# grantjr1842/delayed-streams-modeling

Measured on AMD Instinct MI355X. Metric: real-time stream throughput, stt-1b-en_fr @ bs=64 per GPU (Mimi encode + LM decode per 80 ms frame), higher is better.
Workload: dtype bf16 weights + bf16 KV, f32 activations as three exact bf16 pieces, f32 accumulate (v_mfma_f32_16x16x32_bf16); 1 GPU; stt-1b-en_fr batch=64 streaming, ring KV cache full (750 frames), Mimi encode + LM decode HIP path; streams_per_gpu=64, parallelism=replicas x1 (independent stream batches, no per-step collective), streams=encoder stream || 2 LM group stream(s)

## Files before the change

### delayed-streams-modeling_amd/csrc/dsm_engine.hip

```cpp
#include <hip/hip_runtime.h>

#include <cmath>
#include <cstdarg>
#include <cstdio>
#include <cstdlib>
#include <cstring>
#include <atomic>
#include <mutex>
#include <shared_mutex>
#include <string>
#include <set>
#include <vector>

#include "../../include/dsm.h"
#include "dsm_config_presets.h"
#include "dsm_kernels.h"
#include "dsm_numerics.h"
#include "dsm_safetensors.h"

static thread_local std::string g_create_error;

#define HIPCHK_E(eng, expr)                                                                         \
  do {                                                                                              \
    hipError_t _e = (expr);                                                                         \
// ... 181 lines not shown
  int attn_nt = 1;
  bool fuse_front = false;
  int smallk_loop = 1;
  int smallk_min_tiles = 1024;
  int smallk_mt = 4;
  int chunk_loop_min_tiles = 384;
  bool bx3u = true;
  bool wk_norm = false;
  int wk_gate_max_chunks = 4;
  bool bx3u_m64 = true;
  bool bx3u_late = true;
  int attn_unr = 0;
  bool attn_small = true;
  int prio_hi = 0;
  bool serialize_groups = false;
  hipEvent_t ev_codes_consumed = nullptr;
  bool codes_consumed_valid = false;
  hipEvent_t ev_join = nullptr, ev_a = nullptr, ev_b = nullptr, ev_c = nullptr, ev_d = nullptr;
  MimiW mimi_w;
  MimiState mimi[2];
  std::atomic<bool> mimi1_ready{false};
  std::mutex mimi1_mu;
  MimiDecState dec;
  float* h_pcm_out = nullptr;
  LmW lm_w;
  LmState lm;
  std::vector<void*> allocs;
  std::string err;
  float* h_pcm = nullptr;
  float* h_pcm1 = nullptr;
  uint8_t* h_mask = nullptr;
  uint32_t *h_codes = nullptr, *h_text = nullptr;
// ... 666 lines not shown
  }
  int MT = a.M > 32 ? 4 : (a.M > 16 ? 2 : 1);
  while (MT > 1 && (long)gx * chunks * ((a.M + 16 * MT - 1) / (16 * MT)) < 256) MT /= 2;
  if (MT == 4 && e->bx3u && e->bx3u_m64 && e->dot_mode == 1 && sizeof(WT) == 2 && chunks > 1 && a.chunk_loop == 0 && a.M <= 64 &&
      (long)gx * chunks <= 256 && EPI == EPI_STORE)
    MT = 2;
  const bool smallk = e->smallk_loop && chunks == 1 && a.chunk_loop == 0 && (long)gx * ((a.M + 63) / 64) >= e->smallk_min_tiles &&
                      !(e->dot_mode == 1 && sizeof(WT) == 2);
  if (smallk && e->smallk_mt < MT) MT = e->smallk_mt;
  auto ok4 = [](const RowMap& m) { return m.ld % 4 == 0 && m.bstride % 4 == 0; };
  a.vec = (a.N % 4 == 0) && (!a.Y || ok4(a.ymap)) && (!a.Y2 || ok4(a.y2map)) && (!a.res || ok4(a.rmap));
  a.ws_ntiles = (((NT - 1) * a.nt_stride) >> 4) + gx * 4;
  const int mtiles = (a.M + 15) / 16;
  if (chunks > 1) {
    const int wsid = e->sid(st);
    size_t need = (size_t)chunks * mtiles * a.ws_ntiles * 256 * sizeof(float);
    if (need > e->gemm_ws_cap[wsid]) {
      if (e->capturing) {
        e->capture_failed = true;
        e->set_error("split-K workspace grew during a graph capture");
        return DSM_ERR_STATE;
      }
      e->ws_gen += 1;
      HIPCHK(hipStreamSynchronize(st));
      if (e->gemm_ws[wsid]) HIPCHK(hipFree(e->gemm_ws[wsid]));
      e->gemm_ws[wsid] = nullptr;
      e->gemm_ws_cap[wsid] = 0;
      void* p = nullptr;
      HIPCHK(hipMalloc(&p, need));
      e->gemm_ws[wsid] = reinterpret_cast<float*>(p);
      e->gemm_ws_cap[wsid] = need;
    }
    a.ws = e->gemm_ws[wsid];
  }
  dim3 grid(gx, chunks, (a.M + 16 * MT - 1) / (16 * MT));
  const bool nt2 = NT == 1 && e->dot_mode == 1 && sizeof(WT) == 2 && e->bx3_nt2 && a.chunk_loop > 1 && MT == 4 &&
                   (EPI == EPI_STORE || EPI == EPI_QKV) && a.N % 128 == 0 && (long)(a.N / 128) * grid.z >= e->bx3_nt2_min;
  if (nt2) {
    grid.x = a.N / 128;
    a.wg_cols = 128;
    a.nt_stride = 64;
  }
  a.ts = e->timeline ? e->dev_ts_slot(e->tag_gemm[e->sid(st)], e->sid(st), 1, 2) : nullptr;
  const int ph = e->prof_begin(e->tag_gemm[e->sid(st)], st);
  const bool bx3 = e->dot_mode == 1 && sizeof(WT) == 2;
  const bool roll = (a.chunk_loop > 1 && e->roll_prefetch) || smallk;
  constexpr int DMAX = LoopDepth<WT, NT>::MAX;
  const bool deep = DMAX == 4 && e->loop_depth == 4 && !smallk;
// ... 202 lines not shown
```

### delayed-streams-modeling_amd/csrc/dsm_engine_api.inc

```

namespace {

template <typename KVT, int HD, int T>
int launch_attn_t(dsm_engine* e, hipStream_t st, float* out, const float* q, const void* k, const void* v,
                  const uint32_t* start_pos, const uint8_t* active, int B, int H, int ctx, int d, const AttnFused& fq) {
  size_t lds = sizeof(float) * ((size_t)T * ctx + 4 * T * HD + 16);
  if ((long)B * H >= 2048 && (size_t)2 * ctx * HD * sizeof(KVT) >= (size_t)256 * 1024) lds += e->attn_lds_pad;
  if (lds > 64 * 1024) {
    static size_t allowed = 0;
    if (lds > allowed) {
      HIPCHK(hipFuncSetAttribute(reinterpret_cast<const void*>(&attn_kernel<KVT, HD, T, 8>), hipFuncAttributeMaxDynamicSharedMemorySize, (int)lds));
      HIPCHK(hipFuncSetAttribute(reinterpret_cast<const void*>(&attn_kernel<KVT, HD, T, 4>), hipFuncAttributeMaxDynamicSharedMemorySize, (int)lds));
      allowed = lds;
    }
  }
  const int tag = e->tag_attn[e->sid(st)];
  if (T == 1 && HD == 64 && ctx <= 32 && e->attn_small) {
    const int ph = e->prof_begin(tag, st);
    hipLaunchKernelGGL((attn_small_kernel<KVT, 64>), dim3((B * H + 3) / 4), dim3(256), 0, st, out, q, reinterpret_cast<const KVT*>(k),
                       reinterpret_cast<const KVT*>(v), start_pos, active, B * H, H, ctx, d, fq);
    e->prof_end(ph, st);
    HIPCHK(hipGetLastError());
    return 0;
  }
// ... 402 lines not shown
  const dsm_asr_config& c = e->cfg;
  LmState& s = e->lm;
  const LmW& w = e->lm_w;
  LmState::Group& grp = s.groups[g];
  const int B = e->B, d = c.lm.d_model, b0 = grp.b0, nb = grp.nb;
  e->tag_gemm[e->sid(st)] = DSM_PROF_GEMM_LM;
  e->tag_attn[e->sid(st)] = DSM_PROF_ATTN_LM;
  uint8_t* gmask = s.gmask + b0;
  float* x = s.x + (size_t)b0 * d;
  const int hid = w.tr.hidden;
  float *xn = s.xn + (size_t)b0 * d, *q = s.q + (size_t)b0 * d, *att = s.att + (size_t)b0 * d, *gg = s.g + (size_t)b0 * hid;
  float* hidden = s.hidden + (size_t)b0 * d;
  int rc;
  if (c.kv_bf16)
    rc = transformer_forward<uint16_t, uint16_t>(e, st, w.tr, grp.view, x, xn, q, att, gg, nb, 1, gmask, nullptr,
                                                 plain_map(1, 1), w.out_norm, hidden, phase);
  else
    rc = transformer_forward<uint16_t, float>(e, st, w.tr, grp.view, x, xn, q, att, gg, nb, 1, gmask, nullptr,
                                              plain_map(1, 1), w.out_norm, hidden, phase);
  if (rc || phase == 1) return rc;
  float* logits = s.logits + (size_t)b0 * c.text_out_vocab_size;
  {
    GemmArgs a = base_args(w.text_linear, hidden, plain_map(nb, d), nb);
    a.Y = logits; a.ymap = plain_map(nb, c.text_out_vocab_size);
    if ((rc = gemm_store<uint16_t>(e, st, a))) return rc;
  }
  if (c.temperature > 0.0f)
    hipLaunchKernelGGL(lm_gumbel_kernel, dim3(nb), dim3(256), 0, st, logits, c.text_out_vocab_size, c.temperature,
                       s.rng_key + (size_t)b0 * 8, s.rng_pos + b0, d_text_out + b0, s.text_token + b0, s.first_step + b0, gmask);
  else
    hipLaunchKernelGGL(lm_argmax_kernel, dim3(nb), dim3(256), 0, st, logits, c.text_out_vocab_size, d_text_out + b0,
                       s.text_token + b0, s.first_step + b0, gmask);
  HIPCHK(hipGetLastError());
  if (c.extra_heads_num > 0 && d_prs_out) {
    const int ehw = c.extra_heads_num * c.extra_heads_dim;
    float* eh = s.eh + (size_t)b0 * ehw;
    GemmArgs a = base_args(w.extra_heads, hidden, plain_map(nb, d), nb);
    a.Y = eh; a.ymap = plain_map(nb, ehw);
    if ((rc = gemm_store<uint16_t>(e, st, a))) return rc;
    int n = nb * c.extra_heads_num;
    hipLaunchKernelGGL(extra_heads_kernel, dim3((n + 255) / 256), dim3(256), 0, st, eh, d_prs_out + b0, nb,
                       c.extra_heads_num, c.extra_heads_dim, B);
    HIPCHK(hipGetLastError());
  }
  return 0;
}

int lm_group_head(dsm_engine* e, hipStream_t st, int g, const uint32_t* d_codes, const uint8_t* d_mask, bool with_prefix) {
  const dsm_asr_config& c = e->cfg;
  LmState& s = e->lm;
  const LmW& w = e->lm_w;
  LmState::Group& grp = s.groups[g];
  const int d = c.lm.d_model, b0 = grp.b0, nb = grp.nb, nc = c.audio_codebooks;
  uint8_t* gmask = s.gmask + b0;
  HIPCHK(hipMemcpyAsync(gmask, d_mask + b0, (size_t)nb, hipMemcpyDeviceToDevice, st));
  float* x = s.x + (size_t)b0 * d;
  hipLaunchKernelGGL(lm_input_kernel, dim3(nb, (d + 511) / 512), dim3(256), 0, st, x, w.text_emb, w.audio_emb,
                     d_codes + (size_t)b0 * nc, s.next_cb + (size_t)b0 * nc, s.text_token + b0, s.first_step + b0, gmask, nc, d,
                     c.audio_vocab_size, (uint32_t)c.audio_vocab_size - 1, (uint32_t)c.text_in_vocab_size - 1);
  hipLaunchKernelGGL(lm_next_codebooks_kernel, dim3((nb * nc + 255) / 256), dim3(256), 0, st, d_codes + (size_t)b0 * nc,
                     s.next_cb + (size_t)b0 * nc, gmask, nb, nc);
  HIPCHK(hipGetLastError());
  if (g > 0) HIPCHK(hipEventRecord(e->ev_grp_in[g], st));
  if (with_prefix)
    if (int rc = lm_group_body(e, st, g, nullptr, nullptr, 1)) return rc;
  return 0;
}

int lm_group_rest(dsm_engine* e, hipStream_t st, int g, uint32_t* d_text_out, float* d_prs_out, bool after_prefix) {
  const uint64_t key = (uint64_t)e->sid(st) ^ ((uint64_t)(uintptr_t)d_text_out << 3) ^ ((uint64_t)(uintptr_t)d_prs_out * 0x9E3779B97F4A7C15ull) ^
                       (after_prefix ? 0x8000000000000000ull : 0ull);
  return run_captured(e, e->g_grp[g], st, key, [&] { return lm_group_body(e, st, g, d_text_out, d_prs_out, after_prefix ? 2 : 0); });
}

int wait_group_inputs(dsm_engine* e) {
  if (!e->grp_busy) return 0;
  for (size_t g = 1; g < e->lm.groups.size(); ++g) HIPCHK(hipStreamWaitEvent(e->s_model, e->ev_grp_in[g], 0));
  return 0;
// ... 186 lines not shown
  for (auto& ps : e->pipe) {
    if (ps.h_pcm) (void)hipHostFree(ps.h_pcm);
    if (ps.h_mask) (void)hipHostFree(ps.h_mask);
    if (ps.ev_done) (void)hipEventDestroy(ps.ev_done);
    if (ps.ev_consumed) (void)hipEventDestroy(ps.ev_consumed);
  }
  for (float* p : e->gemm_ws)
    if (p) (void)hipFree(p);
  if (e->h_pcm) (void)hipHostFree(e->h_pcm);
  if (e->h_pcm1) (void)hipHostFree(e->h_pcm1);
  if (e->h_mask) (void)hipHostFree(e->h_mask);
  if (e->h_codes) (void)hipHostFree(e->h_codes);
  if (e->h_text) (void)hipHostFree(e->h_text);
  if (e->h_prs) (void)hipHostFree(e->h_prs);
  if (e->h_pcm_out) (void)hipHostFree(e->h_pcm_out);
  for (hipEvent_t ev : {e->ev_join, e->ev_codes_consumed, e->ev_a, e->ev_b, e->ev_c, e->ev_d})
    if (ev) (void)hipEventDestroy(ev);
  for (auto& r : e->prof_recs) { (void)hipEventDestroy(r.a); (void)hipEventDestroy(r.b); }
  for (hipEvent_t ev : e->prof_pool) (void)hipEventDestroy(ev);
  for (int g = 0; g < dsm_engine::kMaxGroups; ++g) {
    if (e->ev_grp_in[g]) (void)hipEventDestroy(e->ev_grp_in[g]);
    if (e->ev_grp_done[g]) (void)hipEventDestroy(e->ev_grp_done[g]);
    if (e->ev_stagger[g]) (void)hipEventDestroy(e->ev_stagger[g]);
    if (e->s_grp[g]) (void)hipStreamDestroy(e->s_grp[g]);
  }
  if (e->ev_fork) (void)hipEventDestroy(e->ev_fork);
  if (e->s_enc) (void)hipStreamDestroy(e->s_enc);
  if (e->s_model) (void)hipStreamDestroy(e->s_model);
  delete e;
}

// ... 95 lines not shown
  if (const char* env = getenv("DSM_WK_GATE_CHUNKS")) e->wk_gate_max_chunks = atoi(env);
  if (const char* env = getenv("DSM_FUSE_FRONT")) e->fuse_front = atoi(env) != 0;
  if (const char* env = getenv("DSM_ATTN_NT")) e->attn_nt = atoi(env);
  if (const char* env = getenv("DSM_SMALLK_LOOP")) e->smallk_loop = atoi(env);
  if (const char* env = getenv("DSM_SMALLK_MIN")) e->smallk_min_tiles = atoi(env);
  if (const char* env = getenv("DSM_SMALLK_MT")) { const int v = atoi(env); if (v == 1 || v == 2 || v == 4) e->smallk_mt = v; }
  if (c.dot_mode == 1) e->attn_lds_pad = 40000;
  if (const char* env = getenv("DSM_ATTN_LDS_PAD")) e->attn_lds_pad = (size_t)atol(env);
  if (const char* env = getenv("DSM_ENC_CUS")) e->enc_cus = atoi(env);
  if (const char* env = getenv("DSM_BX3_NT2")) e->bx3_nt2 = atoi(env) != 0;
  if (const char* env = getenv("DSM_BX3_NT2_MIN")) e->bx3_nt2_min = atoi(env);
  if (const char* env = getenv("DSM_LM_CUS_EXCL")) e->lm_cus_excl = atoi(env) != 0;
  if (int rc = make_stream(e, &e->s_enc, prio_lo, 1)) return rc;
  if (int rc = make_stream(e, &e->s_model, prio_hi, 2)) return rc;
  HIPCHK(hipEventCreateWithFlags(&e->ev_join, hipEventDisableTiming));
  HIPCHK(hipEventCreateWithFlags(&e->ev_codes_consumed, hipEventDisableTiming));
  HIPCHK(hipEventCreate(&e->ev_a));
  HIPCHK(hipEventCreate(&e->ev_b));
  HIPCHK(hipEventCreate(&e->ev_c));
  HIPCHK(hipEventCreate(&e->ev_d));
  const int B = batch_size, d = c.lm.d_model;
  if (attach_arena) {
    e->arena = const_cast<char*>(reinterpret_cast<const char*>(attach_arena));
    e->arena_size = attach_bytes;
    e->arena_owned = false;
    e->manifest.assign(attach_manifest, attach_manifest + attach_manifest_bytes);
    e->manifest_pos = 0;
    e->arena_off = 0;
    e->wmode = dsm_engine::W_ATTACH;
    if (int rc = load_all_weights(e, nullptr, nullptr)) return rc;
    if (e->arena_off != e->arena_size || e->manifest_pos != e->manifest.size()) {
// ... 79 lines not shown
      int nb = std::min(blocks * 16, B - b0);
      LmState::Group& grp = s.groups[g];
      grp.b0 = b0;
      grp.nb = nb;
      grp.view = s.tr;
      for (int l = 0; l < c.lm.num_layers; ++l) {
        grp.view.k[l] = (char*)s.tr.k[l] + (size_t)b0 * H * c.lm.context * hd * kv_elem;
        grp.view.v[l] = (char*)s.tr.v[l] + (size_t)b0 * H * c.lm.context * hd * kv_elem;
      }
      grp.view.pos = s.tr.pos + b0;
      grp.view.idx = s.tr.idx + b0;
      grp.view.start_pos = s.tr.start_pos + b0;
      grp.view.widx = s.tr.widx + b0;
      grp.view.rope_cs = s.tr.rope_cs + (size_t)b0 * hd;
      b0 += nb;
      if (g > 0) {
        if (int rc = make_stream(e, &e->s_grp[g], e->prio_hi, 2)) return rc;
        HIPCHK(hipEventCreateWithFlags(&e->ev_grp_in[g], hipEventDisableTiming));
        HIPCHK(hipEventCreateWithFlags(&e->ev_grp_done[g], hipEventDisableTiming));
      }
    }
    HIPCHK(hipEventCreateWithFlags(&e->ev_fork, hipEventDisableTiming));
    for (int g = 0; g + 1 < G; ++g) HIPCHK(hipEventCreateWithFlags(&e->ev_stagger[g], hipEventDisableTiming));
  }
  {
    long n = (long)B * c.audio_codebooks;
    hipLaunchKernelGGL(fill_u32_kernel, dim3((unsigned)((n + 255) / 256)), dim3(256), 0, e->s_model, s.next_cb,
                       (uint32_t)c.audio_vocab_size - 1, n);
    hipLaunchKernelGGL(fill_u32_kernel, dim3((unsigned)((B + 255) / 256)), dim3(256), 0, e->s_model, s.text_token,
                       (uint32_t)c.text_in_vocab_size - 1, (long)B);
    HIPCHK(hipGetLastError());
    HIPCHK(hipMemsetAsync(s.first_step, 1, B, e->s_model));
  }
// ... 404 lines not shown
  std::lock_guard<std::mutex> lk(e->err_mu);
  snprintf(out->capture_error, sizeof out->capture_error, "%s", e->capture_error.c_str());
}

int dsm_get_metrics(dsm_engine* e, dsm_metrics* out) {
  if (!e || !out) return DSM_ERR_INVALID;
  *out = e->metrics;
  fill_graph_metrics(e, out);
  return 0;
}

int dsm_mimi_encode_step_dev(dsm_engine* e, const float* d_pcm, const uint8_t* d_mask, uint32_t* d_codes_out) {
  if (!e || !d_pcm || !d_mask) return DSM_ERR_INVALID;
  HIPCHK(hipSetDevice(e->device));
  ApiShared api(e);
  if (e->codes_consumed_valid) HIPCHK(hipStreamWaitEvent(e->s_enc, e->ev_codes_consumed, 0));
  if (int rc = upload_pcm(e, 0, e->s_enc, d_pcm, hipMemcpyDeviceToDevice)) return rc;
  HIPCHK(hipMemcpyAsync(e->mimi[0].mask, d_mask, (size_t)e->B, hipMemcpyDeviceToDevice, e->s_enc));
  if (int rc = mimi_encode(e, 0, e->s_enc)) return rc;
  if (d_codes_out)
    HIPCHK(hipMemcpyAsync(d_codes_out, e->mimi[0].codes, sizeof(uint32_t) * (size_t)e->B * e->cfg.mimi.quantizer_n_q,
                          hipMemcpyDeviceToDevice, e->s_enc));
  HIPCHK(hipEventRecord(e->ev_join, e->s_enc));
  e->metrics.steps_encode += 1;
  return 0;
}

int dsm_asr_step_tokens_dev(dsm_engine* e, const uint32_t* d_codes, const uint8_t* d_mask, uint32_t* d_text_tokens_out,
                            float* d_vad_prs_out) {
  if (!e || !d_mask) return DSM_ERR_INVALID;
  HIPCHK(hipSetDevice(e->device));
  ApiShared api(e);
  if (int rc = wait_group_inputs(e)) return rc;
  HIPCHK(hipMemcpyAsync(e->lm.mask, d_mask, (size_t)e->B, hipMemcpyDeviceToDevice, e->s_model));
  const uint32_t* codes = d_codes;
  if (!codes) {
    HIPCHK(hipStreamWaitEvent(e->s_model, e->ev_join, 0));
    HIPCHK(hipMemcpyAsync(e->lm.codes_in, e->mimi[0].codes, sizeof(uint32_t) * (size_t)e->B * e->cfg.audio_codebooks,
                          hipMemcpyDeviceToDevice, e->s_model));
    HIPCHK(hipEventRecord(e->ev_codes_consumed, e->s_model));
    e->codes_consumed_valid = true;
    codes = e->lm.codes_in;
  }
  if (int rc = lm_step(e, e->s_model, codes, e->lm.mask, d_text_tokens_out ? d_text_tokens_out : e->lm.text_out,
                       e->cfg.extra_heads_num > 0 ? (d_vad_prs_out ? d_vad_prs_out : e->lm.prs) : nullptr))
    return rc;
  e->metrics.steps_lm += 1;
  e->model_step_idx += 1;
  return 0;
}

int dsm_asr_step_pcm_dev(dsm_engine* e, const float* d_pcm, const uint8_t* d_mask, uint32_t* d_codes_out,
                         uint32_t* d_text_tokens_out, float* d_vad_prs_out) {
  if (!e || !d_pcm || !d_mask) return DSM_ERR_INVALID;
  HIPCHK(hipSetDevice(e->device));
  if (int rc = ensure_model_side_mimi(e)) return rc;
  ApiShared api(e);
  hipStream_t st = e->s_model;
  if (int rc = wait_group_inputs(e)) return rc;
// ... 192 lines not shown
```

### delayed-streams-modeling_amd/csrc/dsm_kernels.h

```cpp
#pragma once
#include <hip/hip_runtime.h>
#include <stdint.h>
#include "dsm_numerics.h"
#include "dsm_sampling.h"

typedef float f32x4 __attribute__((ext_vector_type(4)));
typedef short dsm_bf16x8 __attribute__((ext_vector_type(8)));

__device__ __forceinline__ float wave_sum64(float v) {
#pragma unroll
  for (int off = 32; off >= 1; off >>= 1) v = v + __shfl_xor(v, off, 64);
  return v;
}

enum { EPI_STORE = 0, EPI_QKV = 1, EPI_GATE = 2, EPI_RVQ = 3 };

struct RowMap {
  long bstride;
  int rpb;
  int ld;
  int toff;
  __host__ __device__ long off(int m) const { return (long)(m / rpb) * bstride + (long)((m % rpb) + toff) * ld; }
};

// ... 27 lines not shown
  float* ws;
  int ws_ntiles;
  int defer_reduce;
  int chunk_loop;
  const float* norm_w;
  const float* norm_b;
  float* norm_out;
  float norm_eps;
  int norm_rms;
  int wk_hint;
  const float* pre_norm_w;
  const float* pre_norm_b;
  float pre_norm_eps;
  int pre_norm_rms;
  unsigned long long* ts;
};

template <typename WT>
__device__ __forceinline__ const WT* dsm_wbase(const GemmArgs& a, const WT* W, int n0, int r, int q) {
  if (sizeof(WT) == 2 && a.wpacked) return W + ((long)(n0 >> 4) * (a.Kpad >> 5)) * 512 + (q * 16 + r) * 8;
  return W + (long)(n0 + r) * a.Kpad + 8 * q;
}
template <typename WT>
__device__ __forceinline__ int dsm_wstep(const GemmArgs& a) { return (sizeof(WT) == 2 && a.wpacked) ? 16 : 1; }

__device__ __forceinline__ void launch_stamp_begin(unsigned long long* ts) {
  if (!ts || threadIdx.x != 0) return;
  const unsigned lin = blockIdx.x + gridDim.x * (blockIdx.y + gridDim.y * blockIdx.z);
  if (lin < 128) atomicMin(&ts[0], wall_clock64());
}
// ... 1243 lines not shown
  }
  __syncthreads();
  if (rope_cs) {
    const int half = hd / 2;
    for (int e = threadIdx.x; e < T * half; e += blockDim.x) {
      int t = e / half, i = e % half;
      float ang = (float)(s_pos_after + (uint32_t)t) * inv_freq[i];
      float s, c;
      dsm_sincosf(ang, &s, &c);
      rope_cs[((long)(b * T + t) * half + i) * 2] = c;
      rope_cs[((long)(b * T + t) * half + i) * 2 + 1] = s;
    }
  }
}

__global__ void lm_input_kernel(float* __restrict__ x, const uint16_t* __restrict__ text_emb,
                                const uint16_t* __restrict__ audio_emb ,
                                const uint32_t* __restrict__ codes , uint32_t* __restrict__ next_cb,
                                const uint32_t* __restrict__ text_token, const uint8_t* __restrict__ first_step,
                                const uint8_t* __restrict__ active, int nc, int d, int audio_vocab,
                                uint32_t pad_tok, uint32_t start_tok) {
  const int b = blockIdx.x;
  __shared__ uint32_t toks[64];
  const bool first = first_step[b] != 0;
  if (threadIdx.x < nc) toks[threadIdx.x] = first ? pad_tok : next_cb[b * nc + threadIdx.x];
  __syncthreads();
  const uint32_t tt = first ? start_tok : text_token[b];
  const int j = (blockIdx.y * blockDim.x + threadIdx.x) * 2;
  if (j < d) {
    uint32_t t2 = *reinterpret_cast<const uint32_t*>(text_emb + (long)tt * d + j);
    float e0 = __uint_as_float(t2 << 16), e1 = __uint_as_float(t2 & 0xFFFF0000u);
    for (int i = 0; i < nc; ++i) {
      uint32_t a2 = *reinterpret_cast<const uint32_t*>(audio_emb + ((long)i * audio_vocab + toks[i]) * d + j);
      e0 = e0 + __uint_as_float(a2 << 16);
      e1 = e1 + __uint_as_float(a2 & 0xFFFF0000u);
    }
    *reinterpret_cast<float2*>(x + (long)b * d + j) = make_float2(e0, e1);
  }
}

__global__ void lm_next_codebooks_kernel(const uint32_t* __restrict__ codes, uint32_t* __restrict__ next_cb,
                                         const uint8_t* __restrict__ active, int B, int nc) {
  const int i = blockIdx.x * blockDim.x + threadIdx.x;
  if (i < B * nc && active[i / nc]) next_cb[i] = codes[i];
}

__device__ inline int block_argmax_first(const float* __restrict__ lg, int V) {
  float bv = -DSM_INF_F;
  int bi = 0x7FFFFFFF;
  for (int j = threadIdx.x; j < V; j += blockDim.x) {
    float v = lg[j];
    if (v > bv || (v == bv && j < bi)) { bv = v; bi = j; }
  }
  __shared__ float sv[256];
  __shared__ int si[256];
  sv[threadIdx.x] = bv;
  si[threadIdx.x] = bi;
  __syncthreads();
  for (int off = blockDim.x / 2; off >= 1; off >>= 1) {
    if ((int)threadIdx.x < off) {
      float ov = sv[threadIdx.x + off];
      int oi = si[threadIdx.x + off];
      if (ov > sv[threadIdx.x] || (ov == sv[threadIdx.x] && oi < si[threadIdx.x])) {
        sv[threadIdx.x] = ov;
        si[threadIdx.x] = oi;
      }
    }
    __syncthreads();
  }
  const int r = si[0] == 0x7FFFFFFF ? 0 : si[0];
  __syncthreads();
  return r;
}

__global__ void lm_argmax_kernel(const float* __restrict__ logits, int V, uint32_t* __restrict__ text_out,
                                 uint32_t* __restrict__ text_token, uint8_t* __restrict__ first_step,
                                 const uint8_t* __restrict__ active) {
  const int b = blockIdx.x;
  const uint32_t tok = (uint32_t)block_argmax_first(logits + (long)b * V, V);
  if (threadIdx.x == 0) {
    text_out[b] = tok;
    if (active[b]) {
      text_token[b] = tok;
      first_step[b] = 0;
    }
  }
}

__global__ void lm_gumbel_kernel(const float* __restrict__ logits, int V, float temperature, const uint32_t* __restrict__ rng_key,
                                 unsigned long long* __restrict__ rng_pos, uint32_t* __restrict__ text_out,
                                 uint32_t* __restrict__ text_token, uint8_t* __restrict__ first_step,
                                 const uint8_t* __restrict__ active) {
  const int b = blockIdx.x;
  const float* lg = logits + (long)b * V;
  uint32_t key[8];
#pragma unroll
  for (int i = 0; i < 8; ++i) key[i] = rng_key[b * 8 + i];
  const unsigned long long pos = rng_pos[b];
  float bv = -DSM_INF_F;
  int bi = 0x7FFFFFFF;
  const int nblk = (V + 15) >> 4;
  for (int blk = threadIdx.x; blk < nblk; blk += blockDim.x) {
    uint32_t w[16];
    dsm_chacha_block(key, (pos >> 4) + (unsigned long long)blk, 12, w);
#pragma unroll
    for (int i = 0; i < 16; ++i) {
      const int j = 16 * blk + i;
      if (j < V) {
        const float v = dsm_gumbel_value(lg[j], w[i], temperature);
        if (v > bv || (v == bv && j < bi)) { bv = v; bi = j; }
      }
    }
  }
  __shared__ float sv[256];
  __shared__ int si[256];
  sv[threadIdx.x] = bv;
  si[threadIdx.x] = bi;
  __syncthreads();
  for (int off = blockDim.x / 2; off >= 1; off >>= 1) {
    if ((int)threadIdx.x < off) {
      const float ov = sv[threadIdx.x + off];
      const int oi = si[threadIdx.x + off];
      if (ov > sv[threadIdx.x] || (ov == sv[threadIdx.x] && oi < si[threadIdx.x])) { sv[threadIdx.x] = ov; si[threadIdx.x] = oi; }
    }
    __syncthreads();
  }
  if (threadIdx.x == 0) {
    const uint32_t tok = si[0] == 0x7FFFFFFF ? 0u : (uint32_t)si[0];
    text_out[b] = tok;
    if (active[b]) {
      text_token[b] = tok;
      first_step[b] = 0;
      rng_pos[b] = pos + 16ull * (unsigned long long)nblk;
    }
  }
}

__global__ void tts_input_kernel(float* __restrict__ x, const uint16_t* __restrict__ text_emb,
                                 const uint16_t* __restrict__ audio_emb ,
                                 const int32_t* __restrict__ tokens, int nc, int d, int audio_vocab) {
  const int b = blockIdx.x;
  __shared__ int32_t toks[72];
  if ((int)threadIdx.x < 1 + nc) toks[threadIdx.x] = tokens[b * (1 + nc) + threadIdx.x];
  __syncthreads();
  const int j = (blockIdx.y * blockDim.x + threadIdx.x) * 2;
  if (j < d) {
    uint32_t t2 = *reinterpret_cast<const uint32_t*>(text_emb + (long)toks[0] * d + j);
    float e0 = __uint_as_float(t2 << 16), e1 = __uint_as_float(t2 & 0xFFFF0000u);
    for (int i = 0; i < nc; ++i) {
      const int32_t t = toks[1 + i];
// ... 247 lines not shown
    lat[(long)b * S + k] = tok;
    const uint32_t nt = (forced[b] && k > 0) ? pad : tok;
    last_tok[b] = nt;
    s_next = nt;
  }
  if (!next.x) return;
  }
  __syncthreads();
  const uint32_t t = s_next;
  for (int j = 0; j < next.rps; ++j) {
    if (j > 0) __syncthreads();
    dep_head_row(next, b * next.rps + j, t, hred);
  }
}

__global__ void extra_heads_kernel(const float* __restrict__ eh , float* __restrict__ prs, int B,
                                   int nh, int dim, int prs_stride ) {
  int i = blockIdx.x * blockDim.x + threadIdx.x;
  if (i >= B * nh) return;
  int b = i / nh, h = i % nh;
  const float* lg = eh + ((long)b * nh + h) * dim;
  float m = lg[0];
  for (int k = 1; k < dim; ++k) m = lg[k] > m ? lg[k] : m;
  float sum = 0.0f, e0 = 0.0f;
  for (int k = 0; k < dim; ++k) {
    float e = dsm_expf(lg[k] - m);
    if (k == 0) e0 = e;
    sum = sum + e;
  }
  prs[(long)h * prs_stride + b] = e0 / sum;
}

struct SeanetFrontArgs {
  const float* cat_init;
  const float *w0, *b0;
  const float *w1, *b1;
  const float *w2, *b2;
  float* cat_ra;
  float* cat_down;
  int ld0, ld1, ld2;
  int T, S0, Sd;
};

template <int TM>
constexpr size_t seanet_front_lds() { return sizeof(float) * ((TM + 2) * 64 + TM * 64 + TM * 32 + (TM + 2 + 7 - 1)); }
// ... 270 lines not shown
```

Measured before the change: 1817 x realtime (stream-seconds of audio per wall second).

## Fuse LM head input, KV bookkeeping, first norm; defer split-K reduce into sampling

Combines the LM input embedding, next-codebook copy, mask copy, position/ring-index update, rope sin/cos and the first layer's pre-norm into one per-row lm_head_kernel. The text and extra-heads GEMMs skip their split-K reduction; the argmax/Gumbel and softmax kernels sum the partial chunks themselves from a shared workspace at offsets set by ws_base. The encoder's code-copy handoff is also dropped: the LM reads Mimi codes directly, and the encoder waits on per-group input events instead. The aim is fewer kernel launches and device copies per step, at the cost of more complex workspace management and heavier sampling kernels.

After: 1813 x realtime (stream-seconds of audio per wall second), median of 2. Within noise of the previous version (-0.2%).

```diff
diff --git a/delayed-streams-modeling_amd/csrc/dsm_engine.hip b/delayed-streams-modeling_amd/csrc/dsm_engine.hip
--- a/delayed-streams-modeling_amd/csrc/dsm_engine.hip
+++ b/delayed-streams-modeling_amd/csrc/dsm_engine.hip
@@ -219,8 +219,7 @@
   bool attn_small = true;
   int prio_hi = 0;
   bool serialize_groups = false;
-  hipEvent_t ev_codes_consumed = nullptr;
-  bool codes_consumed_valid = false;
+  std::atomic<bool> enc_codes_read{false};
   hipEvent_t ev_join = nullptr, ev_a = nullptr, ev_b = nullptr, ev_c = nullptr, ev_d = nullptr;
   MimiW mimi_w;
   MimiState mimi[2];
@@ -917,7 +916,7 @@
   const int mtiles = (a.M + 15) / 16;
   if (chunks > 1) {
     const int wsid = e->sid(st);
-    size_t need = (size_t)chunks * mtiles * a.ws_ntiles * 256 * sizeof(float);
+    size_t need = ((size_t)a.ws_base + (size_t)chunks * mtiles * a.ws_ntiles * 256) * sizeof(float);
     if (need > e->gemm_ws_cap[wsid]) {
       if (e->capturing) {
         e->capture_failed = true;
@@ -926,15 +925,20 @@
       }
       e->ws_gen += 1;
       HIPCHK(hipStreamSynchronize(st));
+      void* p = nullptr;
+      HIPCHK(hipMalloc(&p, need));
+      if (a.ws_base > 0 && e->gemm_ws[wsid])
+      {
+        HIPCHK(hipMemcpyAsync(p, e->gemm_ws[wsid], std::min((size_t)a.ws_base * sizeof(float), e->gemm_ws_cap[wsid]), hipMemcpyDeviceToDevice, st));
+        HIPCHK(hipStreamSynchronize(st));
+      }
       if (e->gemm_ws[wsid]) HIPCHK(hipFree(e->gemm_ws[wsid]));
       e->gemm_ws[wsid] = nullptr;
       e->gemm_ws_cap[wsid] = 0;
-      void* p = nullptr;
-      HIPCHK(hipMalloc(&p, need));
       e->gemm_ws[wsid] = reinterpret_cast<float*>(p);
       e->gemm_ws_cap[wsid] = need;
     }
-    a.ws = e->gemm_ws[wsid];
+    a.ws = e->gemm_ws[wsid] + a.ws_base;
   }
   dim3 grid(gx, chunks, (a.M + 16 * MT - 1) / (16 * MT));
   const bool nt2 = NT == 1 && e->dot_mode == 1 && sizeof(WT) == 2 && e->bx3_nt2 && a.chunk_loop > 1 && MT == 4 &&
diff --git a/delayed-streams-modeling_amd/csrc/dsm_engine_api.inc b/delayed-streams-modeling_amd/csrc/dsm_engine_api.inc
--- a/delayed-streams-modeling_amd/csrc/dsm_engine_api.inc
+++ b/delayed-streams-modeling_amd/csrc/dsm_engine_api.inc
@@ -440,33 +440,72 @@
   int rc;
   if (c.kv_bf16)
     rc = transformer_forward<uint16_t, uint16_t>(e, st, w.tr, grp.view, x, xn, q, att, gg, nb, 1, gmask, nullptr,
-                                                 plain_map(1, 1), w.out_norm, hidden, phase);
+                                                 plain_map(1, 1), w.out_norm, hidden, phase, nullptr, true);
   else
     rc = transformer_forward<uint16_t, float>(e, st, w.tr, grp.view, x, xn, q, att, gg, nb, 1, gmask, nullptr,
-                                              plain_map(1, 1), w.out_norm, hidden, phase);
+                                              plain_map(1, 1), w.out_norm, hidden, phase, nullptr, true);
   if (rc || phase == 1) return rc;
-  float* logits = s.logits + (size_t)b0 * c.text_out_vocab_size;
+  const int V = c.text_out_vocab_size, mt16 = (nb + 15) / 16;
+  float* logits = s.logits + (size_t)b0 * V;
+  LogitSrc tsrc{}, hsrc{};
+  tsrc.rps = hsrc.rps = 1;
+  long ws_used = 0;
+  bool tdefer = false;
   {
     GemmArgs a = base_args(w.text_linear, hidden, plain_map(nb, d), nb);
-    a.Y = logits; a.ymap = plain_map(nb, c.text_out_vocab_size);
+    a.Y = logits; a.ymap = plain_map(nb, V);
+    a.defer_reduce = (a.Kpad > DSM_KC && a.K % 32 == 0 && !a.bias && V % 4 == 0) ? 1 : 0;
     if ((rc = gemm_store<uint16_t>(e, st, a))) return rc;
-  }
-  if (c.temperature > 0.0f)
-    hipLaunchKernelGGL(lm_gumbel_kernel, dim3(nb), dim3(256), 0, st, logits, c.text_out_vocab_size, c.temperature,
-                       s.rng_key + (size_t)b0 * 8, s.rng_pos + b0, d_text_out + b0, s.text_token + b0, s.first_step + b0, gmask);
-  else
-    hipLaunchKernelGGL(lm_argmax_kernel, dim3(nb), dim3(256), 0, st, logits, c.text_out_vocab_size, d_text_out + b0,
-                       s.text_token + b0, s.first_step + b0, gmask);
-  HIPCHK(hipGetLastError());
-  if (c.extra_heads_num > 0 && d_prs_out) {
+    if (a.defer_reduce) {
+      tdefer = true;
+      tsrc.ld = (long)a.ws_ntiles * 16;
+      tsrc.cstride = (long)mt16 * 16 * tsrc.ld;
+      tsrc.chunks = (a.Kpad + DSM_KC - 1) / DSM_KC;
+      tsrc.store = logits;
+      ws_used = tsrc.chunks * tsrc.cstride;
+    } else {
+      tsrc.rows = logits;
+    }
+  }
+  const bool heads = c.extra_heads_num > 0 && d_prs_out;
+  if (heads) {
     const int ehw = c.extra_heads_num * c.extra_heads_dim;
     float* eh = s.eh + (size_t)b0 * ehw;
     GemmArgs a = base_args(w.extra_heads, hidden, plain_map(nb, d), nb);
     a.Y = eh; a.ymap = plain_map(nb, ehw);
+    a.defer_reduce = (a.Kpad > DSM_KC && a.K % 32 == 0 && !a.bias) ? 1 : 0;
+    a.ws_base = ws_used;
     if ((rc = gemm_store<uint16_t>(e, st, a))) return rc;
-    int n = nb * c.extra_heads_num;
-    hipLaunchKernelGGL(extra_heads_kernel, dim3((n + 255) / 256), dim3(256), 0, st, eh, d_prs_out + b0, nb,
-                       c.extra_heads_num, c.extra_heads_dim, B);
+    if (a.defer_reduce) {
+      hsrc.ws = a.ws;
+      hsrc.ld = (long)a.ws_ntiles * 16;
+      hsrc.cstride = (long)mt16 * 16 * hsrc.ld;
+      hsrc.chunks = (a.Kpad + DSM_KC - 1) / DSM_KC;
+      hsrc.store = eh;
+    } else {
+      hsrc.rows = eh;
+    }
+  }
+  if (tdefer) tsrc.ws = e->gemm_ws[e->sid(st)];
+  const size_t lds = sizeof(float) * (size_t)((V + 3) & ~3);
+  if (lds > 160 * 1024) {
+    e->set_error("text_out_vocab_size=%d: a logits row does not fit in LDS", V);
+    return DSM_ERR_INVALID;
+  }
+  if (lds > 64 * 1024) {
+    static size_t allowed = 0;
+    if (lds > allowed) {
+      HIPCHK(hipFuncSetAttribute(reinterpret_cast<const void*>(&lm_text_kernel), hipFuncAttributeMaxDynamicSharedMemorySize, (int)lds));
+      allowed = lds;
+    }
+  }
+  hipLaunchKernelGGL(lm_text_kernel, dim3(nb), dim3(V >= 4096 ? 1024 : 256), lds, st, tsrc, V, c.temperature, s.rng_key + (size_t)b0 * 8,
+                     s.rng_pos + b0, d_text_out + b0, s.text_token + b0, s.first_step + b0, gmask);
+  HIPCHK(hipGetLastError());
+  if (heads) {
+    const int n = c.extra_heads_num * c.extra_heads_dim;
+    hipLaunchKernelGGL(lm_extra_heads_kernel, dim3(nb), dim3(n > 64 ? 256 : 64), sizeof(float) * (size_t)n, st, hsrc,
+                       d_prs_out + b0, c.extra_heads_num, c.extra_heads_dim, B);
     HIPCHK(hipGetLastError());
   }
   return 0;
@@ -477,17 +516,31 @@
   LmState& s = e->lm;
   const LmW& w = e->lm_w;
   LmState::Group& grp = s.groups[g];
+  const dsm_transformer_config& tc = w.tr.cfg;
   const int d = c.lm.d_model, b0 = grp.b0, nb = grp.nb, nc = c.audio_codebooks;
-  uint8_t* gmask = s.gmask + b0;
-  HIPCHK(hipMemcpyAsync(gmask, d_mask + b0, (size_t)nb, hipMemcpyDeviceToDevice, st));
-  float* x = s.x + (size_t)b0 * d;
-  hipLaunchKernelGGL(lm_input_kernel, dim3(nb, (d + 511) / 512), dim3(256), 0, st, x, w.text_emb, w.audio_emb,
-                     d_codes + (size_t)b0 * nc, s.next_cb + (size_t)b0 * nc, s.text_token + b0, s.first_step + b0, gmask, nc, d,
-                     c.audio_vocab_size, (uint32_t)c.audio_vocab_size - 1, (uint32_t)c.text_in_vocab_size - 1);
-  hipLaunchKernelGGL(lm_next_codebooks_kernel, dim3((nb * nc + 255) / 256), dim3(256), 0, st, d_codes + (size_t)b0 * nc,
-                     s.next_cb + (size_t)b0 * nc, gmask, nb, nc);
+  if (nc > 64 || d % 4 != 0 || d > 1024 * DSM_ROW_ITS) {
+    e->set_error("lm_head_kernel: audio_codebooks=%d (at most 64) d_model=%d (a multiple of 4, at most %d)", nc, d, 1024 * DSM_ROW_ITS);
+    return DSM_ERR_INVALID;
+  }
+  LmHeadArgs h;
+  h.mask_in = d_mask + b0; h.gmask = s.gmask + b0;
+  h.codes = d_codes + (size_t)b0 * nc; h.next_cb = s.next_cb + (size_t)b0 * nc;
+  h.text_token = s.text_token + b0; h.first_step = s.first_step + b0;
+  h.text_emb = w.text_emb; h.audio_emb = w.audio_emb;
+  h.x = s.x + (size_t)b0 * d; h.xn = s.xn + (size_t)b0 * d;
+  h.nc = nc; h.d = d; h.audio_vocab = c.audio_vocab_size;
+  h.pad_tok = (uint32_t)c.audio_vocab_size - 1; h.start_tok = (uint32_t)c.text_in_vocab_size - 1;
+  h.pos = grp.view.pos; h.idx = grp.view.idx; h.start_pos = grp.view.start_pos; h.widx = grp.view.widx;
+  h.rope_cs = tc.positional_embedding == 1 ? grp.view.rope_cs : nullptr;
+  h.inv_freq = w.tr.inv_freq;
+  h.ctx = tc.context; h.hd = d / tc.num_heads; h.rope_before = w.tr.rope_pos_before ? 1 : 0;
+  h.nw = w.tr.layers[0].n1w; h.nb = w.tr.layers[0].n1b;
+  h.eps = tc.norm == 1 ? 1e-8f : 1e-5f; h.rms = tc.norm;
+  if (d <= 1024) hipLaunchKernelGGL(lm_head_kernel<1>, dim3(nb), dim3(256), 0, st, h);
+  else if (d <= 2048) hipLaunchKernelGGL(lm_head_kernel<2>, dim3(nb), dim3(512), 0, st, h);
+  else hipLaunchKernelGGL(lm_head_kernel<4>, dim3(nb), dim3(1024), 0, st, h);
   HIPCHK(hipGetLastError());
-  if (g > 0) HIPCHK(hipEventRecord(e->ev_grp_in[g], st));
+  HIPCHK(hipEventRecord(e->ev_grp_in[g], st));
   if (with_prefix)
     if (int rc = lm_group_body(e, st, g, nullptr, nullptr, 1)) return rc;
   return 0;
@@ -704,7 +757,7 @@
   if (e->h_text) (void)hipHostFree(e->h_text);
   if (e->h_prs) (void)hipHostFree(e->h_prs);
   if (e->h_pcm_out) (void)hipHostFree(e->h_pcm_out);
-  for (hipEvent_t ev : {e->ev_join, e->ev_codes_consumed, e->ev_a, e->ev_b, e->ev_c, e->ev_d})
+  for (hipEvent_t ev : {e->ev_join, e->ev_a, e->ev_b, e->ev_c, e->ev_d})
     if (ev) (void)hipEventDestroy(ev);
   for (auto& r : e->prof_recs) { (void)hipEventDestroy(r.a); (void)hipEventDestroy(r.b); }
   for (hipEvent_t ev : e->prof_pool) (void)hipEventDestroy(ev);
@@ -830,7 +883,6 @@
   if (int rc = make_stream(e, &e->s_enc, prio_lo, 1)) return rc;
   if (int rc = make_stream(e, &e->s_model, prio_hi, 2)) return rc;
   HIPCHK(hipEventCreateWithFlags(&e->ev_join, hipEventDisableTiming));
-  HIPCHK(hipEventCreateWithFlags(&e->ev_codes_consumed, hipEventDisableTiming));
   HIPCHK(hipEventCreate(&e->ev_a));
   HIPCHK(hipEventCreate(&e->ev_b));
   HIPCHK(hipEventCreate(&e->ev_c));
@@ -940,9 +992,9 @@
       grp.view.widx = s.tr.widx + b0;
       grp.view.rope_cs = s.tr.rope_cs + (size_t)b0 * hd;
       b0 += nb;
+      HIPCHK(hipEventCreateWithFlags(&e->ev_grp_in[g], hipEventDisableTiming));
       if (g > 0) {
         if (int rc = make_stream(e, &e->s_grp[g], e->prio_hi, 2)) return rc;
-        HIPCHK(hipEventCreateWithFlags(&e->ev_grp_in[g], hipEventDisableTiming));
         HIPCHK(hipEventCreateWithFlags(&e->ev_grp_done[g], hipEventDisableTiming));
       }
     }
@@ -1377,7 +1429,8 @@
   if (!e || !d_pcm || !d_mask) return DSM_ERR_INVALID;
   HIPCHK(hipSetDevice(e->device));
   ApiShared api(e);
-  if (e->codes_consumed_valid) HIPCHK(hipStreamWaitEvent(e->s_enc, e->ev_codes_consumed, 0));
+  if (e->enc_codes_read)
+    for (size_t g = 0; g < e->lm.groups.size(); ++g) HIPCHK(hipStreamWaitEvent(e->s_enc, e->ev_grp_in[g], 0));
   if (int rc = upload_pcm(e, 0, e->s_enc, d_pcm, hipMemcpyDeviceToDevice)) return rc;
   HIPCHK(hipMemcpyAsync(e->mimi[0].mask, d_mask, (size_t)e->B, hipMemcpyDeviceToDevice, e->s_enc));
   if (int rc = mimi_encode(e, 0, e->s_enc)) return rc;
@@ -1394,18 +1447,13 @@
   if (!e || !d_mask) return DSM_ERR_INVALID;
   HIPCHK(hipSetDevice(e->device));
   ApiShared api(e);
-  if (int rc = wait_group_inputs(e)) return rc;
-  HIPCHK(hipMemcpyAsync(e->lm.mask, d_mask, (size_t)e->B, hipMemcpyDeviceToDevice, e->s_model));
   const uint32_t* codes = d_codes;
   if (!codes) {
     HIPCHK(hipStreamWaitEvent(e->s_model, e->ev_join, 0));
-    HIPCHK(hipMemcpyAsync(e->lm.codes_in, e->mimi[0].codes, sizeof(uint32_t) * (size_t)e->B * e->cfg.audio_codebooks,
-                          hipMemcpyDeviceToDevice, e->s_model));
-    HIPCHK(hipEventRecord(e->ev_codes_consumed, e->s_model));
-    e->codes_consumed_valid = true;
-    codes = e->lm.codes_in;
-  }
-  if (int rc = lm_step(e, e->s_model, codes, e->lm.mask, d_text_tokens_out ? d_text_tokens_out : e->lm.text_out,
+    codes = e->mimi[0].codes;
+    e->enc_codes_read = true;
+  }
+  if (int rc = lm_step(e, e->s_model, codes, d_mask, d_text_tokens_out ? d_text_tokens_out : e->lm.text_out,
                        e->cfg.extra_heads_num > 0 ? (d_vad_prs_out ? d_vad_prs_out : e->lm.prs) : nullptr))
     return rc;
   e->metrics.steps_lm += 1;
diff --git a/delayed-streams-modeling_amd/csrc/dsm_kernels.h b/delayed-streams-modeling_amd/csrc/dsm_kernels.h
--- a/delayed-streams-modeling_amd/csrc/dsm_kernels.h
+++ b/delayed-streams-modeling_amd/csrc/dsm_kernels.h
@@ -65,6 +65,7 @@
   float pre_norm_eps;
   int pre_norm_rms;
   unsigned long long* ts;
+  long ws_base;
 };
 
 template <typename WT>
@@ -1338,37 +1339,6 @@
   }
 }
 
-__global__ void lm_input_kernel(float* __restrict__ x, const uint16_t* __restrict__ text_emb,
-                                const uint16_t* __restrict__ audio_emb ,
-                                const uint32_t* __restrict__ codes , uint32_t* __restrict__ next_cb,
-                                const uint32_t* __restrict__ text_token, const uint8_t* __restrict__ first_step,
-                                const uint8_t* __restrict__ active, int nc, int d, int audio_vocab,
-                                uint32_t pad_tok, uint32_t start_tok) {
-  const int b = blockIdx.x;
-  __shared__ uint32_t toks[64];
-  const bool first = first_step[b] != 0;
-  if (threadIdx.x < nc) toks[threadIdx.x] = first ? pad_tok : next_cb[b * nc + threadIdx.x];
-  __syncthreads();
-  const uint32_t tt = first ? start_tok : text_token[b];
-  const int j = (blockIdx.y * blockDim.x + threadIdx.x) * 2;
-  if (j < d) {
-    uint32_t t2 = *reinterpret_cast<const uint32_t*>(text_emb + (long)tt * d + j);
-    float e0 = __uint_as_float(t2 << 16), e1 = __uint_as_float(t2 & 0xFFFF0000u);
-    for (int i = 0; i < nc; ++i) {
-      uint32_t a2 = *reinterpret_cast<const uint32_t*>(audio_emb + ((long)i * audio_vocab + toks[i]) * d + j);
-      e0 = e0 + __uint_as_float(a2 << 16);
-      e1 = e1 + __uint_as_float(a2 & 0xFFFF0000u);
-    }
-    *reinterpret_cast<float2*>(x + (long)b * d + j) = make_float2(e0, e1);
-  }
-}
-
-__global__ void lm_next_codebooks_kernel(const uint32_t* __restrict__ codes, uint32_t* __restrict__ next_cb,
-                                         const uint8_t* __restrict__ active, int B, int nc) {
-  const int i = blockIdx.x * blockDim.x + threadIdx.x;
-  if (i < B * nc && active[i / nc]) next_cb[i] = codes[i];
-}
-
 __device__ inline int block_argmax_first(const float* __restrict__ lg, int V) {
   float bv = -DSM_INF_F;
   int bi = 0x7FFFFFFF;
@@ -1395,69 +1365,6 @@
   const int r = si[0] == 0x7FFFFFFF ? 0 : si[0];
   __syncthreads();
   return r;
-}
-
-__global__ void lm_argmax_kernel(const float* __restrict__ logits, int V, uint32_t* __restrict__ text_out,
-                                 uint32_t* __restrict__ text_token, uint8_t* __restrict__ first_step,
-                                 const uint8_t* __restrict__ active) {
-  const int b = blockIdx.x;
-  const uint32_t tok = (uint32_t)block_argmax_first(logits + (long)b * V, V);
-  if (threadIdx.x == 0) {
-    text_out[b] = tok;
-    if (active[b]) {
-      text_token[b] = tok;
-      first_step[b] = 0;
-    }
-  }
-}
-
-__global__ void lm_gumbel_kernel(const float* __restrict__ logits, int V, float temperature, const uint32_t* __restrict__ rng_key,
-                                 unsigned long long* __restrict__ rng_pos, uint32_t* __restrict__ text_out,
-                                 uint32_t* __restrict__ text_token, uint8_t* __restrict__ first_step,
-                                 const uint8_t* __restrict__ active) {
-  const int b = blockIdx.x;
-  const float* lg = logits + (long)b * V;
-  uint32_t key[8];
-#pragma unroll
-  for (int i = 0; i < 8; ++i) key[i] = rng_key[b * 8 + i];
-  const unsigned long long pos = rng_pos[b];
-  float bv = -DSM_INF_F;
-  int bi = 0x7FFFFFFF;
-  const int nblk = (V + 15) >> 4;
-  for (int blk = threadIdx.x; blk < nblk; blk += blockDim.x) {
-    uint32_t w[16];
-    dsm_chacha_block(key, (pos >> 4) + (unsigned long long)blk, 12, w);
-#pragma unroll
-    for (int i = 0; i < 16; ++i) {
-      const int j = 16 * blk + i;
-      if (j < V) {
-        const float v = dsm_gumbel_value(lg[j], w[i], temperature);
-        if (v > bv || (v == bv && j < bi)) { bv = v; bi = j; }
-      }
-    }
-  }
-  __shared__ float sv[256];
-  __shared__ int si[256];
-  sv[threadIdx.x] = bv;
-  si[threadIdx.x] = bi;
-  __syncthreads();
-  for (int off = blockDim.x / 2; off >= 1; off >>= 1) {
-    if ((int)threadIdx.x < off) {
-      const float ov = sv[threadIdx.x + off];
-      const int oi = si[threadIdx.x + off];
-      if (ov > sv[threadIdx.x] || (ov == sv[threadIdx.x] && oi < si[threadIdx.x])) { sv[threadIdx.x] = ov; si[threadIdx.x] = oi; }
-    }
-    __syncthreads();
-  }
-  if (threadIdx.x == 0) {
-    const uint32_t tok = si[0] == 0x7FFFFFFF ? 0u : (uint32_t)si[0];
-    text_out[b] = tok;
-    if (active[b]) {
-      text_token[b] = tok;
-      first_step[b] = 0;
-      rng_pos[b] = pos + 16ull * (unsigned long long)nblk;
-    }
-  }
 }
 
 __global__ void tts_input_kernel(float* __restrict__ x, const uint16_t* __restrict__ text_emb,
@@ -1735,21 +1642,249 @@
   }
 }
 
-__global__ void extra_heads_kernel(const float* __restrict__ eh , float* __restrict__ prs, int B,
-                                   int nh, int dim, int prs_stride ) {
-  int i = blockIdx.x * blockDim.x + threadIdx.x;
-  if (i >= B * nh) return;
-  int b = i / nh, h = i % nh;
-  const float* lg = eh + ((long)b * nh + h) * dim;
-  float m = lg[0];
-  for (int k = 1; k < dim; ++k) m = lg[k] > m ? lg[k] : m;
-  float sum = 0.0f, e0 = 0.0f;
-  for (int k = 0; k < dim; ++k) {
-    float e = dsm_expf(lg[k] - m);
-    if (k == 0) e0 = e;
-    sum = sum + e;
-  }
-  prs[(long)h * prs_stride + b] = e0 / sum;
+struct LmHeadArgs {
+  const uint8_t* mask_in;
+  uint8_t* gmask;
+  const uint32_t* codes;
+  uint32_t* next_cb;
+  const uint32_t* text_token;
+  const uint8_t* first_step;
+  const uint16_t* text_emb;
+  const uint16_t* audio_emb;
+  float* x;
+  float* xn;
+  int nc, d, audio_vocab;
+  uint32_t pad_tok, start_tok;
+  uint32_t* pos;
+  uint32_t* idx;
+  uint32_t* start_pos;
+  uint32_t* widx;
+  float* rope_cs;
+  const float* inv_freq;
+  int ctx, hd, rope_before;
+  const float* nw;
+  const float* nb;
+  float eps;
+  int rms;
+};
+template <int ITS>
+__global__ __launch_bounds__(256 * ITS) void lm_head_kernel(LmHeadArgs h) {
+  __shared__ float red[8];
+  __shared__ float carry[2][256];
+  __shared__ uint32_t toks[64];
+  __shared__ uint32_t s_pos_after;
+  const int b = blockIdx.x, tid = threadIdx.x, nc = h.nc, d = h.d;
+  const bool on = h.mask_in[b] != 0;
+  const bool first = h.first_step[b] != 0;
+  if (tid < nc) toks[tid] = first ? h.pad_tok : h.next_cb[b * nc + tid];
+  if (tid == 0) {
+    h.gmask[b] = on ? 1 : 0;
+    uint32_t p = h.pos[b];
+    const uint32_t i = h.idx[b], p0 = p;
+    h.start_pos[b] = p;
+    h.widx[b] = on ? (uint32_t)(i % h.ctx) : i;
+    if (on) {
+      h.pos[b] = p + 1;
+      h.idx[b] = (uint32_t)((i + 1) % h.ctx);
+      p += 1;
+    }
+    s_pos_after = h.rope_before ? p0 : p;
+  }
+  __syncthreads();
+  if (tid < nc && on) h.next_cb[b * nc + tid] = h.codes[b * nc + tid];
+  if (h.rope_cs) {
+    const int half = h.hd / 2;
+    for (int i = tid; i < half; i += blockDim.x) {
+      const float ang = (float)s_pos_after * h.inv_freq[i];
+      float s, c;
+      dsm_sincosf(ang, &s, &c);
+      h.rope_cs[((long)b * half + i) * 2] = c;
+      h.rope_cs[((long)b * half + i) * 2 + 1] = s;
+    }
+  }
+  const uint32_t tt = first ? h.start_tok : h.text_token[b];
+  const int it = tid >> 8, t = tid & 255;
+  const int i = it * 1024 + 4 * t;
+  const bool live = i < d;
+  const int ic = live ? i : 0;
+  const uint2 t4 = *reinterpret_cast<const uint2*>(h.text_emb + (long)tt * d + ic);
+  float o[4] = {__uint_as_float(t4.x << 16), __uint_as_float(t4.x & 0xFFFF0000u), __uint_as_float(t4.y << 16),
+                __uint_as_float(t4.y & 0xFFFF0000u)};
+#pragma unroll 16
+  for (int k = 0; k < nc; ++k) {
+    const uint2 a4 = *reinterpret_cast<const uint2*>(h.audio_emb + ((long)k * h.audio_vocab + toks[k]) * d + ic);
+    o[0] = o[0] + __uint_as_float(a4.x << 16);
+    o[1] = o[1] + __uint_as_float(a4.x & 0xFFFF0000u);
+    o[2] = o[2] + __uint_as_float(a4.y << 16);
+    o[3] = o[3] + __uint_as_float(a4.y & 0xFFFF0000u);
+  }
+  if (live) *reinterpret_cast<float4*>(h.x + (long)b * d + i) = make_float4(o[0], o[1], o[2], o[3]);
+  float s = 0.0f, s2 = 0.0f;
+#pragma unroll
+  for (int k = 0; k < ITS; ++k) {
+    if (it == k) {
+      if (k > 0) { s = carry[0][t]; s2 = carry[1][t]; }
+      if (live) {
+        s = s + o[0]; s2 = DSM_FMAF(o[0], o[0], s2);
+        s = s + o[1]; s2 = DSM_FMAF(o[1], o[1], s2);
+        s = s + o[2]; s2 = DSM_FMAF(o[2], o[2], s2);
+        s = s + o[3]; s2 = DSM_FMAF(o[3], o[3], s2);
+      }
+      if (k + 1 < ITS) { carry[0][t] = s; carry[1][t] = s2; }
+    }
+    if (k + 1 < ITS) __syncthreads();
+  }
+  if (it == ITS - 1) {
+    const int lane = t & 63, wave = t >> 6;
+    s = wave_sum64(s);
+    s2 = wave_sum64(s2);
+    if (lane == 0) { red[wave] = s; red[4 + wave] = s2; }
+  }
+  __syncthreads();
+  s = ((red[0] + red[1]) + red[2]) + red[3];
+  s2 = ((red[4] + red[5]) + red[6]) + red[7];
+  if (live) {
+    float mm = 1.f, mean = 0.f, inv = 0.f;
+    if (h.rms) {
+      mm = sqrtf(s2 / (float)d + h.eps);
+    } else {
+      mean = s / (float)d;
+      float var = s2 / (float)d - mean * mean;
+      inv = 1.0f / sqrtf(var + h.eps);
+    }
+    const float4 wv = *reinterpret_cast<const float4*>(h.nw + i);
+    float4 r;
+    if (h.rms) {
+      r.x = (o[0] / mm) * wv.x; r.y = (o[1] / mm) * wv.y; r.z = (o[2] / mm) * wv.z; r.w = (o[3] / mm) * wv.w;
+    } else {
+      const float4 bv = *reinterpret_cast<const float4*>(h.nb + i);
+      r.x = ((o[0] - mean) * inv) * wv.x + bv.x; r.y = ((o[1] - mean) * inv) * wv.y + bv.y;
+      r.z = ((o[2] - mean) * inv) * wv.z + bv.z; r.w = ((o[3] - mean) * inv) * wv.w + bv.w;
+    }
+    *reinterpret_cast<float4*>(h.xn + (long)b * d + i) = r;
+  }
+}
+
+__device__ __forceinline__ uint32_t block_argmax_pairs(float bv, int bi, float* sv, int* si) {
+#pragma unroll
+  for (int off = 32; off >= 1; off >>= 1) {
+    const float ov = __shfl_xor(bv, off, 64);
+    const int oi = __shfl_xor(bi, off, 64);
+    if (ov > bv || (ov == bv && oi < bi)) { bv = ov; bi = oi; }
+  }
+  if ((threadIdx.x & 63) == 0) { sv[threadIdx.x >> 6] = bv; si[threadIdx.x >> 6] = bi; }
+  __syncthreads();
+  bv = sv[0]; bi = si[0];
+  for (int w = 1; w < (int)(blockDim.x >> 6); ++w) {
+    const float ov = sv[w];
+    const int oi = si[w];
+    if (ov > bv || (ov == bv && oi < bi)) { bv = ov; bi = oi; }
+  }
+  return bi == 0x7FFFFFFF ? 0u : (uint32_t)bi;
+}
+__global__ __launch_bounds__(1024) void lm_text_kernel(LogitSrc src, int V, float temperature, const uint32_t* __restrict__ rng_key,
+                                                        unsigned long long* __restrict__ rng_pos, uint32_t* __restrict__ text_out,
+                                                        uint32_t* __restrict__ text_token, uint8_t* __restrict__ first_step,
+                                                        const uint8_t* __restrict__ active) {
+  extern __shared__ __attribute__((aligned(16))) unsigned char smem[];
+  __shared__ float sv[16];
+  __shared__ int si[16];
+  float* logits = reinterpret_cast<float*>(smem);
+  const int b = blockIdx.x, nthr = blockDim.x;
+  if (src.ws || (V & 3) == 0) {
+    for (int j = 4 * (int)threadIdx.x; j < V; j += 8 * nthr) {
+      const int j1 = j + 4 * nthr;
+      const bool two = j1 < V;
+      const f32x4 o0 = logit4(src, b, V, j);
+      const f32x4 o1 = logit4(src, b, V, two ? j1 : j);
+      if (src.ws && src.store) {
+        *reinterpret_cast<f32x4*>(src.store + (long)b * V + j) = o0;
+        if (two) *reinterpret_cast<f32x4*>(src.store + (long)b * V + j1) = o1;
+      }
+      *reinterpret_cast<f32x4*>(logits + j) = o0;
+      if (two) *reinterpret_cast<f32x4*>(logits + j1) = o1;
+    }
+  } else {
+    for (int j = threadIdx.x; j < V; j += nthr) logits[j] = src.rows[(long)b * V + j];
+  }
+  __syncthreads();
+  float bv = -DSM_INF_F;
+  int bi = 0x7FFFFFFF;
+  unsigned long long pos = 0;
+  const int nblk = (V + 15) >> 4;
+  if (!(temperature > 0.0f)) {
+    for (int j = threadIdx.x; j < V; j += nthr) {
+      const float v = logits[j];
+      if (v > bv || (v == bv && j < bi)) { bv = v; bi = j; }
+    }
+  } else {
+    uint32_t key[8];
+#pragma unroll
+    for (int i = 0; i < 8; ++i) key[i] = rng_key[b * 8 + i];
+    pos = rng_pos[b];
+    for (int blk = threadIdx.x; blk < nblk; blk += nthr) {
+      uint32_t w[16];
+      dsm_chacha_block(key, (pos >> 4) + (unsigned long long)blk, 12, w);
+#pragma unroll
+      for (int i = 0; i < 16; ++i) {
+        const int j = 16 * blk + i;
+        if (j < V) {
+          const float v = dsm_gumbel_value(logits[j], w[i], temperature);
+          if (v > bv || (v == bv && j < bi)) { bv = v; bi = j; }
+        }
+      }
+    }
+  }
+  const uint32_t tok = block_argmax_pairs(bv, bi, sv, si);
+  if (threadIdx.x == 0) {
+    text_out[b] = tok;
+    if (active[b]) {
+      text_token[b] = tok;
+      first_step[b] = 0;
+      if (temperature > 0.0f) rng_pos[b] = pos + 16ull * (unsigned long long)nblk;
+    }
+  }
+}
+
+__global__ void lm_extra_heads_kernel(LogitSrc src, float* __restrict__ prs, int nh, int dim, int prs_stride ) {
+  extern __shared__ __attribute__((aligned(16))) unsigned char smem[];
+  float* lg = reinterpret_cast<float*>(smem);
+  const int b = blockIdx.x, n = nh * dim;
+  for (int j = threadIdx.x; j < n; j += blockDim.x) {
+    float t;
+    if (src.ws) {
+      const float* p = src.ws + (long)b * src.ld + j;
+      t = p[0];
+      for (int c0 = 1; c0 < src.chunks; c0 += 8) {
+        float v[8];
+#pragma unroll
+        for (int u = 0; u < 8; ++u) {
+          const int c = c0 + u < src.chunks ? c0 + u : src.chunks - 1;
+          v[u] = p[c * src.cstride];
+        }
+#pragma unroll
+        for (int u = 0; u < 8; ++u)
+          if (c0 + u < src.chunks) t = t + v[u];
+      }
+      if (src.store) src.store[(long)b * n + j] = t;
+    } else {
+      t = src.rows[(long)b * n + j];
+    }
+    lg[j] = t;
+  }
+  __syncthreads();
+  for (int h = threadIdx.x; h < nh; h += blockDim.x) {
+    const float* l = lg + h * dim;
+    float m = l[0];
+    for (int k = 1; k < dim; ++k) m = l[k] > m ? l[k] : m;
+    float sum = 0.0f, e0 = 0.0f;
+    for (int k = 0; k < dim; ++k) {
+      float e = dsm_expf(l[k] - m);
+      if (k == 0) e0 = e;
+      sum = sum + e;
+    }
+    prs[(long)h * prs_stride + b] = e0 / sum;
+  }
 }
 
 struct SeanetFrontArgs {
```
